# andewx/dieselfluid

Hardware: AMD Instinct MI355X
Metric: M particle-steps/sec, 16M-particle WCSPH dam-break; % HBM roofline (higher is better)
Workload: dtype f32; 1 GPU; WCSPH dam-break, 16003008 particles (n3=252), h=2dx, uniform-grid neighbours, density + pressure/viscosity force + integrate + walls, math=fast; particles=16003008, parallelism=single GPU

## Files before the change

dieselfluid_amd/csrc/kernels_skin.hpp:

```cpp
#pragma once

#include "kernels_tiled.hpp"

namespace dsl {

constexpr int kLEntries = 8;
constexpr int kLMaxChunks = 12;
constexpr int kLMaxEntries = kLMaxChunks * kLEntries - 1;
constexpr int kLBlock = 512;
constexpr unsigned int kLGlobal = 0xffffu;
constexpr float kSkinTauSteps = 16.0f;
constexpr int kLQuads = 14;
static_assert(kTRows * kLQuads <= kLBlock, "one quad per lane");
#ifndef DSL_LIST_WALK
#define DSL_LIST_WALK 2
#endif
constexpr int kListWalk = DSL_LIST_WALK;
constexpr int force_list_waves(bool want_v) { return (kListWalk & 2) != 0 && !want_v ? 6 : 4; }

__global__ void k_skin_decide(SkinState* st) {
  const float d = __builtin_sqrtf(__uint_as_float(st->disp2_bits)) * (1.0f + 1.0e-6f);
  const bool rb = st->force != 0 || !(d <= st->budget);
  st->rebuild = rb ? 1 : 0;
  if (st->unlisted * 64 > st->n_live) st->give_up = 1;
  if (rb) {
    st->ids_sel ^= 1;
    st->n_rebuilds += 1;
    st->unlisted = 0;
    st->fields_own = st->fields_padded = 0u;
    const float vmax = __builtin_sqrtf(__uint_as_float(st->vmax2_bits)) * (1.0f + 1.0e-6f);
    float tau = 0.0f;
    if (st->predict > 0.0f && vmax > 0.0f && vmax < 3.0e38f) tau = fminf(st->predict * st->budget / vmax, kSkinTauSteps * st->dt);
    st->tau = tau;
  }
  st->disp = d;
  st->force = 0;
  st->disp2_bits = 0u;
  st->vmax2_bits = 0u;
  st->n_steps += 1;
  st->history = (st->history << 1) | (rb ? 1u : 0u);
  if (st->n_steps >= 16 && __builtin_popcount(st->history & 0xffffu) >= 5) st->give_up = 1;
}

__device__ __forceinline__ unsigned int pad_entry(const TileMeta& m) { return (unsigned int)(m.row_lds[1] - kTPad) << 4; }

__global__ __launch_bounds__(kLBlock) void k_list_build_v1(DevConsts c, TileGrid tg, const int* __restrict__ desc_of,
                                                        const int* __restrict__ n_tiles, const int* __restrict__ desc,
                                                        const unsigned int* __restrict__ nmask, int mstride,
                                                        uint4* __restrict__ lists, int lstride, SkinState* st,
                                                        SkinGate gate, CSoa3 p, float wide_thr) {
  if (gate.closed()) return;
  __shared__ TileMeta metas[2];
  constexpr int kLStaged = 8;
  __shared__ uint4 held[kLStaged][kLBlock];
  __shared__ unsigned int tile_fields[2];
  const int tid = threadIdx.x;
  if (tid < 2) tile_fields[tid] = 0u;
  TileFeed feed(desc_of, *n_tiles);
  int di = 0;
  bool have = feed.pop(di);
  if (have) tile_meta_store(metas[0], tile_meta_request(desc, di));
  for (int cur = 0; have; cur ^= 1) {
    const TileMeta& m = metas[cur];
    sync_lds();
    have = feed.pop(di);
    int table_word = 0;
    if (have) table_word = tile_meta_request(desc, di);
    const int ntarg = m.tprefix[kTB * kTB];
    const unsigned int pad = pad_entry(m);
    if (m.overflow != 0 && tid == 0) atomicAdd(&st->unlisted, ntarg);
    for_each_target<true, kLBlock>(ntarg, tid, tid, [&](auto shared_c, int t, int sub, int k) {
      constexpr bool SHARED = decltype(shared_c)::value;
      if (SHARED && sub != 0) return;
      const TileTarget tt = tile_target(m, t);
      const int g = tt.g;
      unsigned int b0 = 0u, b1 = 0u, b2 = 0u, b3 = 0u;
      int n = 0;
      auto push = [&](unsigned int entry) {
        b0 = __builtin_amdgcn_alignbit(b1, b0, 16);
        b1 = __builtin_amdgcn_alignbit(b2, b1, 16);
        b2 = __builtin_amdgcn_alignbit(b3, b2, 16);
        b3 = (b3 >> 16) | (entry << 16);
        n += 1;
        if ((n & (kLEntries - 1)) == 0) {
          const int ch = (n >> 3) - 1;
          if (ch < kLStaged) held[ch][tid] = make_uint4(b0, b1, b2, b3);
          else if (ch < kLMaxChunks) lists[(size_t)ch * lstride + g] = make_uint4(b0, b1, b2, b3);
        }
      };
      auto emit = [&](int rec) {
        if (rec != tt.own) push((unsigned int)rec << 4);
      };
      const bool masks = m.overflow == 0;
      if (masks) {
        int rj[9], rje[9];
        unsigned int w1[9], w2[9];
#pragma unroll
        for (int ri = 0; ri < 9; ++ri) {
          tile_run(m, tt.srow + (ri / 3 - 1) * kTH + (ri % 3 - 1), tt.lx, rj[ri], rje[ri]);
          const int len = rje[ri] - rj[ri];
          w1[ri] = (len > 0 && len <= 64) ? nmask[(size_t)ri * mstride + g] : 0u;
          w2[ri] = (len > 32 && len <= 64) ? nmask[(size_t)(kMaskHigh + ri) * mstride + g] : 0u;
        }
        push(0u);
#pragma unroll
        for (int ri = 0; ri < 9; ++ri) {
          const int j = rj[ri], je = rje[ri], len = je - j;
          if (len > 64) {
            const int rr = tt.srow + (ri / 3 - 1) * kTH + (ri % 3 - 1);
            const int g0 = m.row_gs[rr] - m.row_lds[rr];
            const float xi = p.x[g], yi = p.y[g], zi = p.z[g];
            for (int r = j; r < je; ++r) {
              const float dx = xi - p.x[g0 + r], dy = yi - p.y[g0 + r], dz = zi - p.z[g0 + r];
              const float tq = __builtin_fmaf(-dist2<true>(dx, dy, dz), c.inv_hh, 1.0f);
              if (tq > wide_thr) emit(r);
            }
            continue;
          }
          unsigned int w = w1[ri];
          int top = j + ((min(len, 32) + 3) & ~3) - 1;
          while (w != 0u) {
            const int b = __builtin_ctz(w);
            w &= w - 1u;
            emit(top - b);
          }
          w = w2[ri];
          top = j + 32 + ((len - 32 + 3) & ~3) - 1;
          while (w != 0u) {
            const int b = __builtin_ctz(w);
            w &= w - 1u;
            emit(top - b);
          }
        }
      }
      const bool fits = masks && n <= kLMaxChunks * kLEntries;
      if (masks && !fits) st->list_overflow = 1;
      int fields = fits ? n : 0;
      const int own_fields = fields;
      if constexpr (!SHARED) {
        int wmax = 0;
#pragma unroll
        for (int bit = 6; bit >= 0; --bit) {
          const int cand = wmax | (1 << bit);
          if (__builtin_amdgcn_ballot_w64(fields >= cand) != 0ull) wmax = cand;
        }
        fields = wmax;
      }
      atomicAdd(&tile_fields[0], (unsigned int)own_fields);
      atomicAdd(&tile_fields[1], (unsigned int)(fits ? fields : 0));
      const int nch = (fields + kLEntries - 1) / kLEntries;
      if (fits)
        while (n < nch * kLEntries) push(pad);
      for (int ch = 0; ch < min(nch, kLStaged); ++ch) {
        uint4 v = held[ch][tid];
        if (ch == 0) v.x = (v.x & 0xffff0000u) | (unsigned int)fields;
        if (fits) lists[(size_t)ch * lstride + g] = v;
      }
      if (!fits) lists[g] = make_uint4(kLGlobal, 0u, 0u, 0u);
    });
    if (have) tile_meta_store(metas[cur ^ 1], table_word);
    sync_lds();
    if (tid == 0) {
      atomicAdd(&st->fields_own, tile_fields[0]);
      atomicAdd(&st->fields_padded, tile_fields[1]);
      tile_fields[0] = tile_fields[1] = 0u;
    }
  }
}

constexpr int kLQueue = 24;
__global__ __launch_bounds__(kLBlock, 4) void k_list_build(DevConsts c, TileGrid tg, const int* __restrict__ desc_of,
                                                        const int* __restrict__ n_tiles, const int* __restrict__ desc,
                                                        const unsigned int* __restrict__ nmask, int mstride,
                                                        uint4* __restrict__ lists, int lstride, SkinState* st,
                                                        SkinGate gate, CSoa3 p, float wide_thr) {
  if (gate.closed()) return;
  __shared__ TileMeta metas[2];
  __shared__ unsigned int qword[kLQueue][kLBlock];
  __shared__ unsigned short qtop[kLQueue][kLBlock];
  __shared__ unsigned int tile_fields[2];
  const int tid = threadIdx.x;
  if (tid < 2) tile_fields[tid] = 0u;
  TileFeed feed(desc_of, *n_tiles);
  int di = 0;
  bool have = feed.pop(di);
  if (have) tile_meta_store(metas[0], tile_meta_request(desc, di));
  for (int cur = 0; have; cur ^= 1) {
    const TileMeta& m = metas[cur];
    sync_lds();
    have = feed.pop(di);
    int table_word = 0;
    if (have) table_word = tile_meta_request(desc, di);
    const int ntarg = m.tprefix[kTB * kTB];
    const unsigned int pad = pad_entry(m);
    if (m.overflow != 0 && tid == 0) atomicAdd(&st->unlisted, ntarg);
    for_each_target<true, kLBlock>(ntarg, tid, tid, [&](auto shared_c, int t, int sub, int k) {
      constexpr bool SHARED = decltype(shared_c)::value;
      if (SHARED && sub != 0) return;
      const TileTarget tt = tile_target(m, t);
      const int g = tt.g;
      const bool masks = m.overflow == 0;
      int nq = 0, total = 0;
      bool too_many = false;
      auto enqueue = [&](unsigned int w, int top) {
        if (w != 0u) {
          if (nq < kLQueue) {
            qword[nq][tid] = w;
            qtop[nq][tid] = (unsigned short)top;
          } else {
            too_many = true;
          }
          nq += 1;
          total += __builtin_popcount(w);
        }
      };
      if (masks) {
        unsigned int run[9], w1[9], w2[9];
        unsigned int unmasked = 0u;
#pragma unroll
        for (int ri = 0; ri < 9; ++ri) {
          run[ri] = (unsigned int)m.run[(tt.srow + (ri / 3 - 1) * kTH + (ri % 3 - 1)) * kTB + tt.lx - 1];
          const int len = (int)(run[ri] >> 16) - (int)(run[ri] & 0xffffu);
          w1[ri] = (len > 0 && len <= 64) ? nmask[(size_t)ri * mstride + g] : 0u;
          w2[ri] = (len > 32 && len <= 64) ? nmask[(size_t)(kMaskHigh + ri) * mstride + g] : 0u;
          if (len > 64) unmasked |= 1u << ri;
        }
#pragma unroll
        for (int ri = 0; ri < 9; ++ri) {
          const int j = (int)(run[ri] & 0xffffu), len = (int)(run[ri] >> 16) - j;
          unsigned int a = w1[ri], b = w2[ri];
          const int top1 = j + ((min(len, 32) + 3) & ~3) - 1;
          const int top2 = j + 32 + ((len - 32 + 3) & ~3) - 1;
          if (ri == 4) {
            const int b1 = top1 - tt.own, b2 = top2 - tt.own;
            if (b1 >= 0 && b1 < 32) a &= ~(1u << b1);
            if (b2 >= 0 && b2 < 32) b &= ~(1u << b2);
          }
          enqueue(a, top1);
          enqueue(b, top2);
        }
        while (unmasked != 0u) {
          const int ri = __builtin_ctz(unmasked);
          unmasked &= unmasked - 1u;
          const int rr = tt.srow + (ri / 3 - 1) * kTH + (ri % 3 - 1);
          int j, je;
          tile_run(m, rr, tt.lx, j, je);
          const int g0 = m.row_gs[rr] - m.row_lds[rr];
          const float xi = p.x[g], yi = p.y[g], zi = p.z[g];
          for (int r0 = j; r0 < je; r0 += 32) {
            unsigned int w = 0u;
            const int top = r0 + 31;
            for (int r = r0; r < min(r0 + 32, je); ++r) {
              const float dx = xi - p.x[g0 + r], dy = yi - p.y[g0 + r], dz = zi - p.z[g0 + r];
              const float tq = __builtin_fmaf(-dist2<true>(dx, dy, dz), c.inv_hh, 1.0f);
              if (tq > wide_thr && r != tt.own) w |= 1u << (top - r);
            }
            enqueue(w, top);
          }
        }
      }
      const int n_own = 1 + total;
      const bool fits = masks && !too_many && n_own <= kLMaxChunks * kLEntries;
      if (masks && !fits) st->list_overflow = 1;
      int fields = fits ? n_own : 0;
      const int own_fields = fields;
      int wmax = 0;
#pragma unroll
      for (int bit = 6; bit >= 0; --bit) {
        const int cand = wmax | (1 << bit);
        if (__builtin_amdgcn_ballot_w64(fields >= cand) != 0ull) wmax = cand;
      }
      if constexpr (!SHARED) fields = fits ? wmax : 0;
      atomicAdd(&tile_fields[0], (unsigned int)own_fields);
      atomicAdd(&tile_fields[1], (unsigned int)fields);
      const int nch = (fields + kLEntries - 1) / kLEntries;
      const int nch_wave = (wmax + kLEntries - 1) / kLEntries;
      unsigned int b0 = 0u, b1 = 0u, b2 = 0u, b3 = 0u;
      unsigned int k0 = 0u, k1 = 0u, k2 = 0u, k3 = 0u;
      int qi = 0;
      unsigned int w = 0u, top = 0u;
      unsigned int wn = (fits && nq > 0) ? qword[0][tid] : 0u, tn = (fits && nq > 0) ? qtop[0][tid] : 0u;
      const int nq_live = fits ? nq : 0;
      for (int it = 0; it < nch_wave * kLEntries; ++it) {
        unsigned int entry = pad;
        if (it == 0) {
          entry = 0u;
        } else {
          if (w == 0u && qi < nq_live) {
            w = wn;
            top = tn;
            qi += 1;
            if (qi < nq_live) {
              wn = qword[qi][tid];
              tn = qtop[qi][tid];
            }
          }
          if (w != 0u) {
            const int b = __builtin_ctz(w);
            w &= w - 1u;
            entry = (top - (unsigned int)b) << 4;
          }
        }
        b0 = __builtin_amdgcn_alignbit(b1, b0, 16);
        b1 = __builtin_amdgcn_alignbit(b2, b1, 16);
        b2 = __builtin_amdgcn_alignbit(b3, b2, 16);
        b3 = (b3 >> 16) | (entry << 16);
        if ((it & (kLEntries - 1)) == kLEntries - 1) {
          const int ch = it >> 3;
          if (ch == 0) {
            k0 = b0, k1 = b1, k2 = b2, k3 = b3;
          } else if (ch < nch) {
            lists[(size_t)ch * lstride + g] = make_uint4(b0, b1, b2, b3);
          }
        }
      }
      if (fits) lists[g] = make_uint4((k0 & 0xffff0000u) | (unsigned int)fields, k1, k2, k3);
      else lists[g] = make_uint4(kLGlobal, 0u, 0u, 0u);
    });
    if (have) tile_meta_store(metas[cur ^ 1], table_word);
    sync_lds();
    if (tid == 0) {
      atomicAdd(&st->fields_own, tile_fields[0]);
      atomicAdd(&st->fields_padded, tile_fields[1]);
      tile_fields[0] = tile_fields[1] = 0u;
    }
  }
}

template <int NF, bool DEALT, class Load4, class Store>
__device__ __forceinline__ void stage_tile(const TileMeta& m, Load4&& load4, Store&& store) {
  if constexpr (DEALT) {
    const int nq = __builtin_amdgcn_readfirstlane((int)m.qprefix[kTRows]);
    auto pass = [&](int base) {
      StageRegs<NF> sr;
      const StageWhere w = stage_issue_dealt<NF>(m, load4, sr, base + (int)threadIdx.x, nq);
      stage_commit_dealt<NF>(sr, w, store);
    };
    pass(0);
    for (int base = kLBlock; base < nq; base += kLBlock) pass(base);
    stage_pads<NF>(m, store, threadIdx.x);
    return;
  }
  const int t = threadIdx.x, r = t / kLQuads, k = t - r * kLQuads;
  if (r >= kTRows) return;
  const int len = m.row_len[r], gs = m.row_gs[r], ls = m.row_lds[r];
  for (int q = k; 4 * q < len; q += kLQuads) {
    float4 v[NF];
    load4(gs + 4 * q, v);
#pragma unroll
    for (int i = 0; i < 4; ++i) {
      if (4 * q + i < len) {
        float rec[NF];
#pragma unroll
        for (int a = 0; a < NF; ++a) rec[a] = f4_at(v[a], i);
        store(ls + 4 * q + i, rec, true);
      }
    }
  }
  const int npad = m.row_lds[r + 1] - ls - len;
  if (k < npad) {
    float rec[NF];
#pragma unroll
    for (int a = 0; a < NF; ++a) rec[a] = 0.0f;
    store(ls + len + k, rec, false);
  }
}

__device__ __forceinline__ const float4& lds_at(const float4* base, unsigned int byte_offset) {
  return *reinterpret_cast<const float4*>(reinterpret_cast<const char*>(base) + byte_offset);
}

struct Chunk {
  unsigned int x, y, z, w;
};
__device__ __forceinline__ Chunk load_chunk(const uint4* __restrict__ lists, size_t index) {
  const uint4 v = lists[index];
  return Chunk{v.x, v.y, v.z, v.w};
}
__device__ __forceinline__ Chunk pad_chunk(unsigned int pad) {
  const unsigned int w = pad | (pad << 16);
  return Chunk{w, w, w, w};
}
__device__ __forceinline__ unsigned int take_count(Chunk& e, unsigned int pad) {
  const unsigned int cnt = e.x & 0xffffu;
  e.x = (e.x & 0xffff0000u) | pad;
  return cnt;
}
__device__ __forceinline__ void loads_issued() {
  asm volatile("" ::: "memory");
  __builtin_amdgcn_sched_barrier(0);
}
typedef unsigned int ListWords __attribute__((ext_vector_type(4)));
typedef const __attribute__((address_space(1))) ListWords* ListPtr;
__device__ __forceinline__ unsigned long long unknown_pointer(const uint4* p) {
  unsigned long long a = reinterpret_cast<unsigned long long>(p);
  asm volatile("" : "+v"(a));
  return a;
}
__device__ __forceinline__ unsigned long long unknown_pointer_uniform(const uint4* p) {
  unsigned long long a = reinterpret_cast<unsigned long long>(p);
  asm volatile("" : "+s"(a));
  return a;
}
struct ChunkRing {
  Chunk c[3];
  unsigned long long next;
  unsigned long long last;
  int lstride, nch;
  __device__ __forceinline__ ChunkRing(const uint4* __restrict__ lists, int lstride_, int g, int nch_, const Chunk& q0,
                                       const Chunk& q1)
      : next(unknown_pointer(lists + (size_t)2 * lstride_ + g)),
        last(unknown_pointer_uniform(lists + (size_t)max(nch_ - 1, 0) * lstride_ + __builtin_amdgcn_readfirstlane(g))),
        lstride(lstride_), nch(nch_) {
    c[0] = q0;
    c[1] = q1;
  }
  __device__ __forceinline__ void request(int ch) {
    if (ch + 2 >= kLMaxChunks) return;
    const ListWords v = *(ListPtr)(ch + 2 < nch ? next : last);
    c[(ch + 2) % 3] = Chunk{v.x, v.y, v.z, v.w};
    next += (unsigned long long)lstride * sizeof(uint4);
  }
  __device__ __forceinline__ const Chunk& at(int ch) const { return c[ch % 3]; }
};
__device__ __forceinline__ int chunks_of(unsigned int cnt) { return cnt == kLGlobal ? 0 : (int)((cnt + kLEntries) >> 3); }

template <class Body>
__device__ __forceinline__ void walk_shared(const uint4* __restrict__ lists, int lstride, int g, unsigned int pad, int sub,
                                            int k, unsigned int fields, Body&& body) {
  const int nch = fields == kLGlobal ? 0 : (int)((fields + kLEntries - 1) >> 3);
  for (int ch = sub; __builtin_amdgcn_ballot_w64(ch < nch) != 0ull; ch += k) {
    Chunk e = pad_chunk(pad);
    if (ch < nch) e = load_chunk(lists, (size_t)ch * lstride + g);
    if (ch == 0) e.x = (e.x & 0xffff0000u) | pad;
    body(e);
  }
}
__device__ __forceinline__ unsigned int shared_fields(const uint4* __restrict__ lists, int g, int sub) {
  unsigned int f = 0u;
  if (sub == 0) f = lists[g].x & 0xffffu;
  return (unsigned int)__shfl((int)f, (int)((threadIdx.x & (kWave - 1)) - sub), kWave);
}

__global__ __launch_bounds__(kLBlock, 4) void k_density_list(DevConsts c, TileGrid tg, const int* __restrict__ desc_of,
                                                             const int* __restrict__ n_tiles, const int* __restrict__ desc,
                                                             const int* __restrict__ cell_start, const SkinState* st,
                                                             CSoa3 pX, CSoa3 pZ, const uint4* __restrict__ lists,
                                                             int lstride, float* __restrict__ rho,
                                                             float* __restrict__ pterm) {
  __shared__ TileMeta metas[2];
  __shared__ float4 A[kTCap];
  const int tid = threadIdx.x;
  const CSoa3 p = st->rebuild ? pZ : pX;
  TileFeed feed(desc_of, *n_tiles);
  int di = 0;
  bool have = feed.pop(di);
  if (have) tile_meta_store(metas[0], tile_meta_request(desc, di));
  for (int cur = 0; have; cur ^= 1) {
    const TileMeta& m = metas[cur];
    sync_lds();
    have = feed.pop(di);
    int table_word = 0;
    if (have) table_word = tile_meta_request(desc, di);
    const int ntarg = m.tprefix[kTB * kTB];
    const bool staged = m.overflow == 0;
    const unsigned int pad = pad_entry(m);
    Chunk q0 = pad_chunk(pad), q1 = q0;
    const bool first_full = ntarg > kLBlock / 2;
    TileTarget tt0{0, 0, 0, 0};
    const int tperm = (tid & ~(kWave - 1)) + b128_group_slot(tid & (kWave - 1));
    if (first_full && tperm < ntarg) {
      tt0 = tile_target(m, tperm);
      q0 = load_chunk(lists, tt0.g);
      q1 = load_chunk(lists, (size_t)lstride + tt0.g);
    }
    if (staged) stage_tile<3, (kStageDealt & 1) != 0>(m, LoadPos4{p}, StoreTileRecord(A, m, c.inv_hh));
    if (have) tile_meta_store(metas[cur ^ 1], table_word);
    sync_lds();
    for_each_target<true, kLBlock>(ntarg, tid, tperm, [&](auto shared_c, int t, int sub, int k) {
      constexpr bool SHARED = decltype(shared_c)::value;
      TileTarget tt;
      unsigned int fields;
      if constexpr (SHARED) {
        tt = tile_target(m, t);
        fields = shared_fields(lists, tt.g, sub);
      } else {
        if (t == tperm) tt = tt0;
        else {
          tt = tile_target(m, t);
          q0 = load_chunk(lists, tt.g);
          q1 = load_chunk(lists, (size_t)lstride + tt.g);
        }
        fields = take_count(q0, pad);
      }
      const int g = tt.g;
      float acc = 0.0f;
      if (staged && fields != kLGlobal) {
        const float4 me = A[tt.own];
        const float two_hh = 2.0f * c.inv_hh;
        const float sx = two_hh * me.x, sy = two_hh * me.y, sz = two_hh * me.z, a0 = 1.0f + me.w;
        float acc0 = 0.0f, acc1 = 0.0f;
        float4 cq[4];
        auto fetch4 = [&](unsigned int w0, unsigned int w1) {
          cq[0] = lds_at(A, w0 & 0xffffu);
          cq[1] = lds_at(A, w0 >> 16);
          cq[2] = lds_at(A, w1 & 0xffffu);
          cq[3] = lds_at(A, w1 >> 16);
        };
        auto sum4 = [&](const float4 (&r)[4]) {
#pragma unroll
          for (int u = 0; u < 4; ++u) {
            const float q = fma_clamp01(r[u].z, sz, __builtin_fmaf(r[u].y, sy, __builtin_fmaf(r[u].x, sx, r[u].w + a0)));
            if (u & 1) acc1 = __builtin_fmaf(q, q, acc1);
            else acc0 = __builtin_fmaf(q, q, acc0);
          }
        };
        if constexpr (SHARED) {
          walk_shared(lists, lstride, g, pad, sub, k, fields, [&](const Chunk& e) {
            fetch4(e.x, e.y);
            float4 c1[4] = {cq[0], cq[1], cq[2], cq[3]};
            fetch4(e.z, e.w);
            sum4(c1);
            sum4(cq);
          });
        } else {
          const int nf = __builtin_amdgcn_readfirstlane((int)fields), nch = (nf + kLEntries - 1) >> 3;
          const uint4* lp = lists + (size_t)2 * lstride + g;
          Chunk e = q0, e1 = q1;
          fetch4(e.x, e.y);
          for (int ch = 0;;) {
            float4 c1[4] = {cq[0], cq[1], cq[2], cq[3]};
            fetch4(e.z, e.w);
            sum4(c1);
            if (8 * ch + 4 >= nf) break;
            const Chunk en = e1;
            if (ch + 2 < nch) e1 = load_chunk(lp, 0);
            lp += lstride;
            float4 c2[4] = {cq[0], cq[1], cq[2], cq[3]};
            fetch4(en.x, en.y);
            sum4(c2);
            e = en;
            ch += 1;
            if (8 * ch >= nf) break;
          }
        }
        acc = acc0 + acc1;
      } else if (sub == 0) {
        const float xi = p.x[g], yi = p.y[g], zi = p.z[g];
        float a = 0.0f;
        for_each_grid_candidate(c, cell_start, xi, yi, zi, [&](int j) {
          if (j == g) return;
          const float dx = xi - p.x[j], dy = yi - p.y[j], dz = zi - p.z[j];
          const float r2 = dist2<true>(dx, dy, dz);
          if (r2 < c.hh) {
            const float q = __builtin_fmaf(-r2, c.inv_hh, 1.0f);
            a = __builtin_fmaf(q, q, a);
          }
        });
        acc = a;
      }
      if constexpr (SHARED) {
        for (int o = 1; o < k; o <<= 1) acc += __shfl_xor(acc, o, kWave);
        if (sub != 0) return;
      }
      acc *= c.mass * c.A;
      rho[g] = acc;
      const float pr = tait_eos<true>(c, acc, c.eos_d0_grad);
      pterm[g] = acc > 0.0f ? dsl_div<true>(pr, acc * acc) : 0.0f;
    });
  }
}

template <bool WANT_G, bool WANT_V, bool QUEUE>
__global__ __launch_bounds__(kLBlock, force_list_waves(WANT_V)) void k_force_list(DevConsts c, TileGrid tg, const int* __restrict__ desc_of,
                                                           const int* __restrict__ n_tiles, const int* __restrict__ desc,
                                                           const int* __restrict__ cell_start, SkinState* st, CSoa3 pX,
                                                           CSoa3 vX, CSoa3 pZ, CSoa3 vZ, CSoa3 pR, const float* __restrict__ rho,
                                                           const float* __restrict__ pterm,
                                                           const uint4* __restrict__ lists, int lstride, Soa3 pout,
                                                           Soa3 vout, DevStats* stats, int* __restrict__ walk_ctr) {
  __shared__ TileMeta metas[2];
  __shared__ float4 A[kTCap];
  __shared__ float4 B[kTCap];
  __shared__ int feed_slot[2];
  const int tid = threadIdx.x;
  const bool rb = st->rebuild != 0;
  const CSoa3 pin = rb ? pZ : pX, vin = rb ? vZ : vX;
  unsigned int vbits = 0u, fbits = 0u, dbits = 0u;
  typename TileSource<QUEUE>::type feed = TileSource<QUEUE>::make(desc_of, *n_tiles, walk_ctr, feed_slot);
  int di = 0;
  bool have = feed.pop(di);
  if (have) tile_meta_store(metas[0], tile_meta_request(desc, di));
  for (int cur = 0; have; cur ^= 1) {
    const TileMeta& m = metas[cur];
    sync_lds();
    have = feed.pop(di);
    int table_word = 0;
    if (have) table_word = tile_meta_request(desc, di);
    const int ntarg = m.tprefix[kTB * kTB];
    const bool staged = m.overflow == 0;
    const unsigned int pad = pad_entry(m);
    Chunk q0 = pad_chunk(pad), q1 = q0;
    const bool first_full = ntarg > kLBlock / 2;
    TileTarget tt0{0, 0, 0, 0};
    const int tperm = (tid & ~(kWave - 1)) + b128_group_slot(tid & (kWave - 1));
    if (first_full && tperm < ntarg) {
      tt0 = tile_target(m, tperm);
      q0 = load_chunk(lists, tt0.g);
      q1 = load_chunk(lists, (size_t)lstride + tt0.g);
    }
    if (staged)
      stage_tile<8, (kStageDealt & 2) != 0>(
          m,
          [&](int gg, float4* o) {
            o[0] = load4u(pin.x + gg);
            o[1] = load4u(pin.y + gg);
            o[2] = load4u(pin.z + gg);
            o[3] = WANT_G ? load4u(pterm + gg) : make_float4(0.f, 0.f, 0.f, 0.f);
            if constexpr (WANT_V) {
              o[4] = load4u(vin.x + gg);
              o[5] = load4u(vin.y + gg);
              o[6] = load4u(vin.z + gg);
              o[7] = load4u(rho + gg);
            } else {
              o[4] = o[5] = o[6] = o[7] = make_float4(0.f, 0.f, 0.f, 0.f);
            }
          },
          [&](int slot, const float* o, bool real) {
            float4 a = make_float4(kFar, kFar, kFar, 0.f), b = make_float4(0.f, 0.f, 0.f, 0.f);
            if (real && o[0] == o[0] && o[1] == o[1] && o[2] == o[2]) {
              a = make_float4(o[0], o[1], o[2], o[3]);
              if constexpr (WANT_V) b = make_float4(o[4], o[5], o[6], o[7] > 0.0f ? __builtin_amdgcn_rcpf(o[7]) : 0.0f);
            }
            A[slot] = a;
            if constexpr (WANT_V) B[slot] = b;
          });
    if (have) tile_meta_store(metas[cur ^ 1], table_word);
    sync_lds();
    for_each_target<true, kLBlock>(ntarg, tid, tperm, [&](auto shared_c, int t, int sub, int k) {
      constexpr bool SHARED = decltype(shared_c)::value;
      TileTarget tt;
      unsigned int fields;
      if constexpr (SHARED) {
        tt = tile_target(m, t);
        fields = shared_fields(lists, tt.g, sub);
      } else {
        if (t == tperm) tt = tt0;
        else {
          tt = tile_target(m, t);
          q0 = load_chunk(lists, tt.g);
          q1 = load_chunk(lists, (size_t)lstride + tt.g);
        }
        fields = take_count(q0, pad);
      }
      const int g = tt.g;
      float px, py, pz, vx, vy, vz;
      float gx = 0.f, gy = 0.f, gz = 0.f, lx_ = 0.f, ly_ = 0.f, lz_ = 0.f, lw_ = 0.f;
      const bool listed = staged && fields != kLGlobal;
      if (listed) {
        const float4 a = A[tt.own];
        px = a.x, py = a.y, pz = a.z;
        const float pti = WANT_G ? a.w : 0.f;
        if (px == kFar) px = py = pz = __uint_as_float(0x7fc00000u);
        if constexpr (WANT_V) {
          const float4 b = B[tt.own];
          vx = b.x, vy = b.y, vz = b.z;
        } else {
          vx = vin.x[g], vy = vin.y[g], vz = vin.z[g];
        }
        if constexpr (WANT_G || WANT_V) {
          const float ninvh = -c.inv_h;
          auto accum = [&](const float4& ra, const float4& rb2) {
            const float dx = ra.x - px, dyy = ra.y - py, dzz = ra.z - pz;
            float r2 = __builtin_fmaf(dzz, dzz, __builtin_fmaf(dyy, dyy, dx * dx));
            r2 = fmaxf(r2, 1.0e-30f);
            const float rinv = __builtin_amdgcn_rsqf(r2);
            const float dist = r2 * rinv;
            const float q = fma1_clamp01_uniform(dist, ninvh);
            if constexpr (WANT_G) {
              const float kk = (q * q) * (pti + ra.w) * rinv;
              gx = __builtin_fmaf(dx, kk, gx);
              gy = __builtin_fmaf(dyy, kk, gy);
              gz = __builtin_fmaf(dzz, kk, gz);
            }
            if constexpr (WANT_V) {
              const float w = q * rb2.w;
              lx_ = __builtin_fmaf(rb2.x, w, lx_);
              ly_ = __builtin_fmaf(rb2.y, w, ly_);
              lz_ = __builtin_fmaf(rb2.z, w, lz_);
              lw_ += w;
            }
          };
          struct Pair1 {
            float4 a, b;
          };
          auto fetch1 = [&](unsigned int off) {
            Pair1 r;
            r.a = lds_at(A, off);
            r.b = r.a;
            if constexpr (WANT_V) r.b = lds_at(B, off);
            return r;
          };
          if constexpr (SHARED) {
            walk_shared(lists, lstride, g, pad, sub, k, fields, [&](const Chunk& e) {
              const unsigned int w[4] = {e.x, e.y, e.z, e.w};
#pragma unroll
              for (int u = 0; u < 4; ++u) {
                const Pair1 r0 = fetch1(w[u] & 0xffffu), r1 = fetch1(w[u] >> 16);
                accum(r0.a, r0.b);
                accum(r1.a, r1.b);
              }
            });
          } else {
            constexpr bool kStraight = (kListWalk & 2) != 0;
            const int nf = __builtin_amdgcn_readfirstlane((int)fields), nch = (nf + kLEntries - 1) >> 3;
            Pair1 p0 = fetch1(q0.x & 0xffffu), p1 = fetch1(q0.x >> 16);
            auto word = [&](unsigned int next_word) {
              Pair1 cu = p0;
              p0 = fetch1(next_word & 0xffffu);
              if constexpr (kStraight) loads_issued();
              accum(cu.a, cu.b);
              cu = p1;
              p1 = fetch1(next_word >> 16);
              if constexpr (kStraight) loads_issued();
              accum(cu.a, cu.b);
            };
            if constexpr (kStraight) {
              ChunkRing ring(lists, lstride, g, nch, q0, q1);
#pragma unroll
              for (int ch = 0; ch < kLMaxChunks; ++ch) {
                ring.request(ch);
                const Chunk& e = ring.at(ch);
                word(e.y);
                if (8 * ch + 2 >= nf) break;
                word(e.z);
                if (8 * ch + 4 >= nf) break;
                word(e.w);
                if (8 * ch + 6 >= nf) break;
                if (ch + 1 == kLMaxChunks) {
                  accum(p0.a, p0.b);
                  accum(p1.a, p1.b);
                  break;
                }
                word(ring.at(ch + 1).x);
                if (8 * ch + 8 >= nf) break;
              }
            } else {
              const uint4* lp = lists + (size_t)2 * lstride + g;
              Chunk e = q0, e1 = q1;
              for (int ch = 0;;) {
                word(e.y);
                if (8 * ch + 2 >= nf) break;
                word(e.z);
                if (8 * ch + 4 >= nf) break;
                word(e.w);
                if (8 * ch + 6 >= nf) break;
                const Chunk en = e1;
                if (ch + 2 < nch) e1 = load_chunk(lp, 0);
                lp += lstride;
                word(en.x);
                e = en;
                ch += 1;
                if (8 * ch >= nf) break;
              }
            }
          }
        }
      } else {
        px = pin.x[g], py = pin.y[g], pz = pin.z[g];
        vx = vin.x[g], vy = vin.y[g], vz = vin.z[g];
        if (sub == 0) {
          float accG[3] = {0.f, 0.f, 0.f}, accV[3] = {0.f, 0.f, 0.f};
          if constexpr (WANT_G || WANT_V)
            force_sweep<true, WANT_G, WANT_V>(c, grid_neigh(cell_start), g, pin, vin, rho, pterm, accG, accV, nullptr, nullptr);
          gx = accG[0], gy = accG[1], gz = accG[2];
          lx_ = accV[0], ly_ = accV[1], lz_ = accV[2];
        }
      }
      if constexpr (SHARED) {
        for (int o = 1; o < k; o <<= 1) {
          gx += __shfl_xor(gx, o, kWave);
          gy += __shfl_xor(gy, o, kWave);
          gz += __shfl_xor(gz, o, kWave);
          lx_ += __shfl_xor(lx_, o, kWave);
          ly_ += __shfl_xor(ly_, o, kWave);
          lz_ += __shfl_xor(lz_, o, kWave);
          lw_ += __shfl_xor(lw_, o, kWave);
        }
        if (sub != 0) return;
      }
      if (listed) {
        if constexpr (WANT_V) {
          lx_ = __builtin_fmaf(-vx, lw_, lx_);
          ly_ = __builtin_fmaf(-vy, lw_, ly_);
          lz_ = __builtin_fmaf(-vz, lw_, lz_);
        }
        const float sg = -c.B;
        gx *= sg;
        gy *= sg;
        gz *= sg;
        const float sv = c.C * c.mass;
        lx_ *= sv;
        ly_ *= sv;
        lz_ *= sv;
      }
      float fx = c.reset[0], fy = c.reset[1], fz = c.reset[2];
      if constexpr (WANT_G) {
        const float dm = rho[g] * c.mass * c.pressure_sign;
        fx = __builtin_fmaf(gx, dm, fx);
        fy = __builtin_fmaf(gy, dm, fy);
        fz = __builtin_fmaf(gz, dm, fz);
      }
      if constexpr (WANT_V) {
        fx = __builtin_fmaf(lx_, c.mu, fx);
        fy = __builtin_fmaf(ly_, c.mu, fy);
        fz = __builtin_fmaf(lz_, c.mu, fz);
      }
      fx += c.ext[0];
      fy += c.ext[1];
      fz += c.ext[2];
      integrate_core(c, fx, fy, fz, px, py, pz, vx, vy, vz, vbits, fbits);
      {
        const float ex = px - pR.x[g], ey = py - pR.y[g], ez = pz - pR.z[g];
        const unsigned int db = nonneg_bits(__builtin_fmaf(ez, ez, __builtin_fmaf(ey, ey, ex * ex)));
        dbits = db > dbits ? db : dbits;
      }
      pout.x[g] = px;
      pout.y[g] = py;
      pout.z[g] = pz;
      vout.x[g] = vx;
      vout.y[g] = vy;
      vout.z[g] = vz;
    });
  }
  feed.finish();
  wave_atomic_max(&stats->max_vel_bits, vbits);
  wave_atomic_max(&stats->max_f_bits, fbits);
  wave_atomic_max(&st->disp2_bits, dbits);
  wave_atomic_max(&st->vmax2_bits, vbits);
}

}
```

Baseline: 8248 M particle-steps/s.

## Pack neighbour list entries as 12-bit indices, ten per 16-byte chunk

```diff
diff --git a/dieselfluid_amd/csrc/kernels_skin.hpp b/dieselfluid_amd/csrc/kernels_skin.hpp
--- a/dieselfluid_amd/csrc/kernels_skin.hpp
+++ b/dieselfluid_amd/csrc/kernels_skin.hpp
@@ -1,17 +1,15 @@
 #pragma once
 
 #include "kernels_tiled.hpp"
+#include "list_chunk.hpp"
 
 namespace dsl {
 
-constexpr int kLEntries = 8;
-constexpr int kLMaxChunks = 12;
-constexpr int kLMaxEntries = kLMaxChunks * kLEntries - 1;
 constexpr int kLBlock = 512;
-constexpr unsigned int kLGlobal = 0xffffu;
 constexpr float kSkinTauSteps = 16.0f;
 constexpr int kLQuads = 14;
 static_assert(kTRows * kLQuads <= kLBlock, "one quad per lane");
+static_assert((unsigned int)kTCap <= kLIndexLimit && (unsigned int)kTCap * sizeof(float4) <= 65536u, "list fields name every staged record");
 #ifndef DSL_LIST_WALK
 #define DSL_LIST_WALK 2
 #endif
@@ -42,7 +40,8 @@
   if (st->n_steps >= 16 && __builtin_popcount(st->history & 0xffffu) >= 5) st->give_up = 1;
 }
 
-__device__ __forceinline__ unsigned int pad_entry(const TileMeta& m) { return (unsigned int)(m.row_lds[1] - kTPad) << 4; }
+__device__ __forceinline__ unsigned int pad_index(const TileMeta& m) { return (unsigned int)(m.row_lds[1] - kTPad); }
+__device__ __forceinline__ unsigned int pad_entry(const TileMeta& m) { return pad_index(m) << 4; }
 
 __global__ __launch_bounds__(kLBlock) void k_list_build_v1(DevConsts c, TileGrid tg, const int* __restrict__ desc_of,
                                                         const int* __restrict__ n_tiles, const int* __restrict__ desc,
@@ -67,29 +66,29 @@
     int table_word = 0;
     if (have) table_word = tile_meta_request(desc, di);
     const int ntarg = m.tprefix[kTB * kTB];
-    const unsigned int pad = pad_entry(m);
+    const unsigned int pad = pad_index(m);
     if (m.overflow != 0 && tid == 0) atomicAdd(&st->unlisted, ntarg);
     for_each_target<true, kLBlock>(ntarg, tid, tid, [&](auto shared_c, int t, int sub, int k) {
       constexpr bool SHARED = decltype(shared_c)::value;
       if (SHARED && sub != 0) return;
       const TileTarget tt = tile_target(m, t);
       const int g = tt.g;
-      unsigned int b0 = 0u, b1 = 0u, b2 = 0u, b3 = 0u;
+      Chunk b{0u, 0u, 0u, 0u};
       int n = 0;
-      auto push = [&](unsigned int entry) {
-        b0 = __builtin_amdgcn_alignbit(b1, b0, 16);
-        b1 = __builtin_amdgcn_alignbit(b2, b1, 16);
-        b2 = __builtin_amdgcn_alignbit(b3, b2, 16);
-        b3 = (b3 >> 16) | (entry << 16);
+      int pos = 0, ch = 0;
+      auto push = [&](unsigned int index) {
+        chunk_push(b, pos, index);
         n += 1;
-        if ((n & (kLEntries - 1)) == 0) {
-          const int ch = (n >> 3) - 1;
-          if (ch < kLStaged) held[ch][tid] = make_uint4(b0, b1, b2, b3);
-          else if (ch < kLMaxChunks) lists[(size_t)ch * lstride + g] = make_uint4(b0, b1, b2, b3);
+        pos += 1;
+        if (pos == kLEntries) {
+          if (ch < kLStaged) held[ch][tid] = make_uint4(b.x, b.y, b.z, b.w);
+          else if (ch < kLMaxChunks) lists[(size_t)ch * lstride + g] = make_uint4(b.x, b.y, b.z, b.w);
+          pos = 0;
+          ch += 1;
         }
       };
       auto emit = [&](int rec) {
-        if (rec != tt.own) push((unsigned int)rec << 4);
+        if (rec != tt.own) push((unsigned int)rec);
       };
       const bool masks = m.overflow == 0;
       if (masks) {
@@ -133,7 +132,7 @@
           }
         }
       }
-      const bool fits = masks && n <= kLMaxChunks * kLEntries;
+      const bool fits = masks && n <= kLMaxEntries + 1;
       if (masks && !fits) st->list_overflow = 1;
       int fields = fits ? n : 0;
       const int own_fields = fields;
@@ -148,15 +147,19 @@
       }
       atomicAdd(&tile_fields[0], (unsigned int)own_fields);
       atomicAdd(&tile_fields[1], (unsigned int)(fits ? fields : 0));
-      const int nch = (fields + kLEntries - 1) / kLEntries;
+      const int nch = chunks_for(fields);
       if (fits)
         while (n < nch * kLEntries) push(pad);
-      for (int ch = 0; ch < min(nch, kLStaged); ++ch) {
-        uint4 v = held[ch][tid];
-        if (ch == 0) v.x = (v.x & 0xffff0000u) | (unsigned int)fields;
-        if (fits) lists[(size_t)ch * lstride + g] = v;
-      }
-      if (!fits) lists[g] = make_uint4(kLGlobal, 0u, 0u, 0u);
+      for (int hc = 0; hc < min(nch, kLStaged); ++hc) {
+        const uint4 v = held[hc][tid];
+        Chunk e{v.x, v.y, v.z, v.w};
+        if (hc == 0) chunk_set_count(e, (unsigned int)fields);
+        if (fits) lists[(size_t)hc * lstride + g] = make_uint4(e.x, e.y, e.z, e.w);
+      }
+      if (!fits) {
+        const Chunk e = chunk_unlisted();
+        lists[g] = make_uint4(e.x, e.y, e.z, e.w);
+      }
     });
     if (have) tile_meta_store(metas[cur ^ 1], table_word);
     sync_lds();
@@ -192,7 +195,7 @@
     int table_word = 0;
     if (have) table_word = tile_meta_request(desc, di);
     const int ntarg = m.tprefix[kTB * kTB];
-    const unsigned int pad = pad_entry(m);
+    const unsigned int pad = pad_index(m);
     if (m.overflow != 0 && tid == 0) atomicAdd(&st->unlisted, ntarg);
     for_each_target<true, kLBlock>(ntarg, tid, tid, [&](auto shared_c, int t, int sub, int k) {
       constexpr bool SHARED = decltype(shared_c)::value;
@@ -260,7 +263,7 @@
         }
       }
       const int n_own = 1 + total;
-      const bool fits = masks && !too_many && n_own <= kLMaxChunks * kLEntries;
+      const bool fits = masks && !too_many && n_own <= kLMaxEntries + 1;
       if (masks && !fits) st->list_overflow = 1;
       int fields = fits ? n_own : 0;
       const int own_fields = fields;
@@ -273,18 +276,19 @@
       if constexpr (!SHARED) fields = fits ? wmax : 0;
       atomicAdd(&tile_fields[0], (unsigned int)own_fields);
       atomicAdd(&tile_fields[1], (unsigned int)fields);
-      const int nch = (fields + kLEntries - 1) / kLEntries;
-      const int nch_wave = (wmax + kLEntries - 1) / kLEntries;
-      unsigned int b0 = 0u, b1 = 0u, b2 = 0u, b3 = 0u;
-      unsigned int k0 = 0u, k1 = 0u, k2 = 0u, k3 = 0u;
+      const int nch = chunks_for(fields);
+      const int nch_wave = chunks_for(wmax);
+      Chunk b{0u, 0u, 0u, 0u};
+      Chunk k0{0u, 0u, 0u, 0u};
+      int pos = 0, ch = 0;
       int qi = 0;
       unsigned int w = 0u, top = 0u;
       unsigned int wn = (fits && nq > 0) ? qword[0][tid] : 0u, tn = (fits && nq > 0) ? qtop[0][tid] : 0u;
       const int nq_live = fits ? nq : 0;
       for (int it = 0; it < nch_wave * kLEntries; ++it) {
-        unsigned int entry = pad;
+        unsigned int index = pad;
         if (it == 0) {
-          entry = 0u;
+          index = 0u;
         } else {
           if (w == 0u && qi < nq_live) {
             w = wn;
@@ -296,26 +300,26 @@
             }
           }
           if (w != 0u) {
-            const int b = __builtin_ctz(w);
+            const int bit = __builtin_ctz(w);
             w &= w - 1u;
-            entry = (top - (unsigned int)b) << 4;
-          }
-        }
-        b0 = __builtin_amdgcn_alignbit(b1, b0, 16);
-        b1 = __builtin_amdgcn_alignbit(b2, b1, 16);
-        b2 = __builtin_amdgcn_alignbit(b3, b2, 16);
-        b3 = (b3 >> 16) | (entry << 16);
-        if ((it & (kLEntries - 1)) == kLEntries - 1) {
-          const int ch = it >> 3;
+            index = top - (unsigned int)bit;
+          }
+        }
+        chunk_push(b, pos, index);
+        pos += 1;
+        if (pos == kLEntries) {
           if (ch == 0) {
-            k0 = b0, k1 = b1, k2 = b2, k3 = b3;
+            k0 = b;
           } else if (ch < nch) {
-            lists[(size_t)ch * lstride + g] = make_uint4(b0, b1, b2, b3);
-          }
-        }
-      }
-      if (fits) lists[g] = make_uint4((k0 & 0xffff0000u) | (unsigned int)fields, k1, k2, k3);
-      else lists[g] = make_uint4(kLGlobal, 0u, 0u, 0u);
+            lists[(size_t)ch * lstride + g] = make_uint4(b.x, b.y, b.z, b.w);
+          }
+          pos = 0;
+          ch += 1;
+        }
+      }
+      if (fits) chunk_set_count(k0, (unsigned int)fields);
+      else k0 = chunk_unlisted();
+      lists[g] = make_uint4(k0.x, k0.y, k0.z, k0.w);
     });
     if (have) tile_meta_store(metas[cur ^ 1], table_word);
     sync_lds();
@@ -370,21 +374,13 @@
   return *reinterpret_cast<const float4*>(reinterpret_cast<const char*>(base) + byte_offset);
 }
 
-struct Chunk {
-  unsigned int x, y, z, w;
-};
 __device__ __forceinline__ Chunk load_chunk(const uint4* __restrict__ lists, size_t index) {
   const uint4 v = lists[index];
   return Chunk{v.x, v.y, v.z, v.w};
 }
-__device__ __forceinline__ Chunk pad_chunk(unsigned int pad) {
+__device__ __forceinline__ Chunk pad_words(unsigned int pad) {
   const unsigned int w = pad | (pad << 16);
   return Chunk{w, w, w, w};
-}
-__device__ __forceinline__ unsigned int take_count(Chunk& e, unsigned int pad) {
-  const unsigned int cnt = e.x & 0xffffu;
-  e.x = (e.x & 0xffff0000u) | pad;
-  return cnt;
 }
 __device__ __forceinline__ void loads_issued() {
   asm volatile("" ::: "memory");
@@ -423,22 +419,42 @@
   }
   __device__ __forceinline__ const Chunk& at(int ch) const { return c[ch % 3]; }
 };
-__device__ __forceinline__ int chunks_of(unsigned int cnt) { return cnt == kLGlobal ? 0 : (int)((cnt + kLEntries) >> 3); }
-
+__device__ __forceinline__ int chunks_of(unsigned int cnt) { return cnt == kLGlobal ? 0 : chunks_for((int)cnt + 1); }
+
+struct Share {
+  unsigned int w[4];
+};
 template <class Body>
 __device__ __forceinline__ void walk_shared(const uint4* __restrict__ lists, int lstride, int g, unsigned int pad, int sub,
                                             int k, unsigned int fields, Body&& body) {
-  const int nch = fields == kLGlobal ? 0 : (int)((fields + kLEntries - 1) >> 3);
-  for (int ch = sub; __builtin_amdgcn_ballot_w64(ch < nch) != 0ull; ch += k) {
-    Chunk e = pad_chunk(pad);
-    if (ch < nch) e = load_chunk(lists, (size_t)ch * lstride + g);
-    if (ch == 0) e.x = (e.x & 0xffff0000u) | pad;
-    body(e);
+  const int nf = fields == kLGlobal ? 0 : (int)fields;
+  const Chunk far_away = pad_words(pad);
+  for (int v = sub; __builtin_amdgcn_ballot_w64(8 * v < nf) != 0ull; v += k) {
+    Share s{{far_away.x, far_away.y, far_away.z, far_away.w}};
+    if constexpr (kLWords == 4) {
+      if (8 * v < nf) {
+        Chunk e = load_chunk(lists, (size_t)v * lstride + g);
+        if (v == 0) chunk_set_first(e, pad);
+        s = Share{{e.x, e.y, e.z, e.w}};
+      }
+    } else if (8 * v < nf) {
+      const int ch = (4 * v) / kLWords, p = 4 * v - ch * kLWords;
+      Chunk e = load_chunk(lists, (size_t)ch * lstride + g);
+      if (ch == 0) chunk_set_first(e, pad);
+      Chunk f = far_away;
+      if (p > 1 && (ch + 1) * kLEntries < nf) f = load_chunk(lists, (size_t)(ch + 1) * lstride + g);
+      const unsigned int t = chunk_tail(e);
+      s.w[0] = p == 0 ? e.x : p == 1 ? e.y : p == 2 ? e.z : p == 3 ? e.w : t;
+      s.w[1] = p == 0 ? e.y : p == 1 ? e.z : p == 2 ? e.w : p == 3 ? t : f.x;
+      s.w[2] = p == 0 ? e.z : p == 1 ? e.w : p == 2 ? t : p == 3 ? f.x : f.y;
+      s.w[3] = p == 0 ? e.w : p == 1 ? t : p == 2 ? f.x : p == 3 ? f.y : f.z;
+    }
+    body(s);
   }
 }
 __device__ __forceinline__ unsigned int shared_fields(const uint4* __restrict__ lists, int g, int sub) {
   unsigned int f = 0u;
-  if (sub == 0) f = lists[g].x & 0xffffu;
+  if (sub == 0) f = chunk_count(load_chunk(lists, g));
   return (unsigned int)__shfl((int)f, (int)((threadIdx.x & (kWave - 1)) - sub), kWave);
 }
 
@@ -465,7 +481,7 @@
     const int ntarg = m.tprefix[kTB * kTB];
     const bool staged = m.overflow == 0;
     const unsigned int pad = pad_entry(m);
-    Chunk q0 = pad_chunk(pad), q1 = q0;
+    Chunk q0 = pad_words(pad), q1 = q0;
     const bool first_full = ntarg > kLBlock / 2;
     TileTarget tt0{0, 0, 0, 0};
     const int tperm = (tid & ~(kWave - 1)) + b128_group_slot(tid & (kWave - 1));
@@ -502,46 +518,93 @@
         float acc0 = 0.0f, acc1 = 0.0f;
         float4 cq[4];
         auto fetch4 = [&](unsigned int w0, unsigned int w1) {
-          cq[0] = lds_at(A, w0 & 0xffffu);
-          cq[1] = lds_at(A, w0 >> 16);
-          cq[2] = lds_at(A, w1 & 0xffffu);
-          cq[3] = lds_at(A, w1 >> 16);
+          cq[0] = lds_at(A, word_lo(w0));
+          cq[1] = lds_at(A, word_hi(w0));
+          cq[2] = lds_at(A, word_lo(w1));
+          cq[3] = lds_at(A, word_hi(w1));
+        };
+        auto sum1 = [&](const float4& r, bool odd) {
+          const float q = fma_clamp01(r.z, sz, __builtin_fmaf(r.y, sy, __builtin_fmaf(r.x, sx, r.w + a0)));
+          if (odd) acc1 = __builtin_fmaf(q, q, acc1);
+          else acc0 = __builtin_fmaf(q, q, acc0);
         };
         auto sum4 = [&](const float4 (&r)[4]) {
 #pragma unroll
-          for (int u = 0; u < 4; ++u) {
-            const float q = fma_clamp01(r[u].z, sz, __builtin_fmaf(r[u].y, sy, __builtin_fmaf(r[u].x, sx, r[u].w + a0)));
-            if (u & 1) acc1 = __builtin_fmaf(q, q, acc1);
-            else acc0 = __builtin_fmaf(q, q, acc0);
-          }
+          for (int u = 0; u < 4; ++u) sum1(r[u], (u & 1) != 0);
         };
         if constexpr (SHARED) {
-          walk_shared(lists, lstride, g, pad, sub, k, fields, [&](const Chunk& e) {
-            fetch4(e.x, e.y);
+          walk_shared(lists, lstride, g, pad, sub, k, fields, [&](const Share& e) {
+            fetch4(e.w[0], e.w[1]);
             float4 c1[4] = {cq[0], cq[1], cq[2], cq[3]};
-            fetch4(e.z, e.w);
-            sum4(c1);
+            cq[0] = lds_at(A, word_lo(e.w[2]));
+            cq[1] = lds_at(A, word_hi(e.w[2]));
+            sum1(c1[0], false);
+            sum1(c1[1], true);
+            loads_issued();
+            cq[2] = lds_at(A, word_lo(e.w[3]));
+            cq[3] = lds_at(A, word_hi(e.w[3]));
+            sum1(c1[2], false);
+            sum1(c1[3], true);
             sum4(cq);
           });
         } else {
-          const int nf = __builtin_amdgcn_readfirstlane((int)fields), nch = (nf + kLEntries - 1) >> 3;
+          const int nf = __builtin_amdgcn_readfirstlane((int)fields), nch = chunks_for(nf);
           const uint4* lp = lists + (size_t)2 * lstride + g;
           Chunk e = q0, e1 = q1;
-          fetch4(e.x, e.y);
-          for (int ch = 0;;) {
-            float4 c1[4] = {cq[0], cq[1], cq[2], cq[3]};
-            fetch4(e.z, e.w);
-            sum4(c1);
-            if (8 * ch + 4 >= nf) break;
-            const Chunk en = e1;
-            if (ch + 2 < nch) e1 = load_chunk(lp, 0);
-            lp += lstride;
-            float4 c2[4] = {cq[0], cq[1], cq[2], cq[3]};
-            fetch4(en.x, en.y);
-            sum4(c2);
-            e = en;
-            ch += 1;
-            if (8 * ch >= nf) break;
+          if constexpr (kLWords == 5) {
+            auto sum3 = [&](const float4 (&r)[3], bool odd) {
+              sum1(r[0], odd);
+              sum1(r[1], !odd);
+              sum1(r[2], odd);
+            };
+            cq[0] = lds_at(A, word_lo(e.x));
+            cq[1] = lds_at(A, word_hi(e.x));
+            cq[2] = lds_at(A, word_lo(e.y));
+            for (int ch = 0, f0 = 0;;) {
+              float4 c1[3] = {cq[0], cq[1], cq[2]};
+              const unsigned int tail = chunk_tail(e);
+              cq[0] = lds_at(A, word_hi(e.y));
+              cq[1] = lds_at(A, word_lo(e.z));
+              cq[2] = lds_at(A, word_hi(e.z));
+              sum3(c1, false);
+              if (f0 + 3 >= nf) break;
+              float4 c2[3] = {cq[0], cq[1], cq[2]};
+              cq[0] = lds_at(A, word_lo(e.w));
+              cq[1] = lds_at(A, word_hi(e.w));
+              cq[2] = lds_at(A, word_lo_clean(tail));
+              cq[3] = lds_at(A, word_hi_clean(tail));
+              sum3(c2, true);
+              if (f0 + 6 >= nf) break;
+              const Chunk en = e1;
+              if (ch + 2 < nch) e1 = load_chunk(lp, 0);
+              lp += lstride;
+              float4 c3[4] = {cq[0], cq[1], cq[2], cq[3]};
+              cq[0] = lds_at(A, word_lo(en.x));
+              cq[1] = lds_at(A, word_hi(en.x));
+              cq[2] = lds_at(A, word_lo(en.y));
+              sum4(c3);
+              e = en;
+              ch += 1;
+              f0 += kLEntries;
+              if (f0 >= nf) break;
+            }
+          } else {
+            fetch4(e.x, e.y);
+            for (int ch = 0;;) {
+              float4 c1[4] = {cq[0], cq[1], cq[2], cq[3]};
+              fetch4(e.z, e.w);
+              sum4(c1);
+              if (8 * ch + 4 >= nf) break;
+              const Chunk en = e1;
+              if (ch + 2 < nch) e1 = load_chunk(lp, 0);
+              lp += lstride;
+              float4 c2[4] = {cq[0], cq[1], cq[2], cq[3]};
+              fetch4(en.x, en.y);
+              sum4(c2);
+              e = en;
+              ch += 1;
+              if (8 * ch >= nf) break;
+            }
           }
         }
         acc = acc0 + acc1;
@@ -600,7 +663,7 @@
     const int ntarg = m.tprefix[kTB * kTB];
     const bool staged = m.overflow == 0;
     const unsigned int pad = pad_entry(m);
-    Chunk q0 = pad_chunk(pad), q1 = q0;
+    Chunk q0 = pad_words(pad), q1 = q0;
     const bool first_full = ntarg > kLBlock / 2;
     TileTarget tt0{0, 0, 0, 0};
     const int tperm = (tid & ~(kWave - 1)) + b128_group_slot(tid & (kWave - 1));
@@ -702,29 +765,30 @@
             return r;
           };
           if constexpr (SHARED) {
-            walk_shared(lists, lstride, g, pad, sub, k, fields, [&](const Chunk& e) {
-              const unsigned int w[4] = {e.x, e.y, e.z, e.w};
+            walk_shared(lists, lstride, g, pad, sub, k, fields, [&](const Share& e) {
 #pragma unroll
               for (int u = 0; u < 4; ++u) {
-                const Pair1 r0 = fetch1(w[u] & 0xffffu), r1 = fetch1(w[u] >> 16);
+                const Pair1 r0 = fetch1(word_lo(e.w[u])), r1 = fetch1(word_hi(e.w[u]));
                 accum(r0.a, r0.b);
                 accum(r1.a, r1.b);
               }
             });
           } else {
             constexpr bool kStraight = (kListWalk & 2) != 0;
-            const int nf = __builtin_amdgcn_readfirstlane((int)fields), nch = (nf + kLEntries - 1) >> 3;
-            Pair1 p0 = fetch1(q0.x & 0xffffu), p1 = fetch1(q0.x >> 16);
-            auto word = [&](unsigned int next_word) {
+            const int nf = __builtin_amdgcn_readfirstlane((int)fields), nch = chunks_for(nf);
+            Pair1 p0 = fetch1(word_lo(q0.x)), p1 = fetch1(word_hi(q0.x));
+            auto word_of = [&](unsigned int next_word, auto clean) {
               Pair1 cu = p0;
-              p0 = fetch1(next_word & 0xffffu);
+              p0 = fetch1(decltype(clean)::value ? word_lo_clean(next_word) : word_lo(next_word));
               if constexpr (kStraight) loads_issued();
               accum(cu.a, cu.b);
               cu = p1;
-              p1 = fetch1(next_word >> 16);
+              p1 = fetch1(decltype(clean)::value ? word_hi_clean(next_word) : word_hi(next_word));
               if constexpr (kStraight) loads_issued();
               accum(cu.a, cu.b);
             };
+            auto word = [&](unsigned int next_word) { word_of(next_word, std::false_type{}); };
+            auto tail = [&](const Chunk& e) { word_of(chunk_tail(e), std::true_type{}); };
             if constexpr (kStraight) {
               ChunkRing ring(lists, lstride, g, nch, q0, q1);
 #pragma unroll
@@ -732,36 +796,45 @@
                 ring.request(ch);
                 const Chunk& e = ring.at(ch);
                 word(e.y);
-                if (8 * ch + 2 >= nf) break;
+                if (kLEntries * ch + 2 >= nf) break;
                 word(e.z);
-                if (8 * ch + 4 >= nf) break;
+                if (kLEntries * ch + 4 >= nf) break;
                 word(e.w);
-                if (8 * ch + 6 >= nf) break;
+                if (kLEntries * ch + 6 >= nf) break;
+                if constexpr (kLWords == 5) {
+                  tail(e);
+                  if (kLEntries * ch + 8 >= nf) break;
+                }
                 if (ch + 1 == kLMaxChunks) {
                   accum(p0.a, p0.b);
                   accum(p1.a, p1.b);
                   break;
                 }
                 word(ring.at(ch + 1).x);
-                if (8 * ch + 8 >= nf) break;
+                if (kLEntries * ch + kLEntries >= nf) break;
               }
             } else {
               const uint4* lp = lists + (size_t)2 * lstride + g;
               Chunk e = q0, e1 = q1;
-              for (int ch = 0;;) {
+              for (int ch = 0, f0 = 0;;) {
                 word(e.y);
-                if (8 * ch + 2 >= nf) break;
+                if (f0 + 2 >= nf) break;
                 word(e.z);
-                if (8 * ch + 4 >= nf) break;
+                if (f0 + 4 >= nf) break;
                 word(e.w);
-                if (8 * ch + 6 >= nf) break;
+                if (f0 + 6 >= nf) break;
+                if constexpr (kLWords == 5) {
+                  tail(e);
+                  if (f0 + 8 >= nf) break;
+                }
                 const Chunk en = e1;
                 if (ch + 2 < nch) e1 = load_chunk(lp, 0);
                 lp += lstride;
                 word(en.x);
                 e = en;
                 ch += 1;
-                if (8 * ch >= nf) break;
+                f0 += kLEntries;
+                if (f0 >= nf) break;
               }
             }
           }
diff --git a/dieselfluid_amd/csrc/list_chunk.hpp b/dieselfluid_amd/csrc/list_chunk.hpp
--- /dev/null
+++ b/dieselfluid_amd/csrc/list_chunk.hpp
@@ -0,0 +1,79 @@
+#pragma once
+
+#ifndef DSL_LIST_BITS
+#define DSL_LIST_BITS 12
+#endif
+#if DSL_LIST_BITS != 12 && DSL_LIST_BITS != 16
+#error "DSL_LIST_BITS is 12 or 16"
+#endif
+
+#if defined(__HIPCC__) || defined(__CUDACC__)
+#define DSL_CHUNK_FN __host__ __device__ __forceinline__
+#else
+#define DSL_CHUNK_FN inline
+#endif
+
+namespace dsl {
+
+constexpr int kListBits = DSL_LIST_BITS;
+constexpr int kLEntries = kListBits == 12 ? 10 : 8;
+constexpr int kLWords = kLEntries / 2;
+constexpr int kLMaxEntries = 95;
+constexpr int kLMaxChunks = (kLMaxEntries + 1 + kLEntries - 1) / kLEntries;
+constexpr unsigned int kLIndexLimit = 4096u;
+constexpr unsigned int kLGlobal = kListBits == 12 ? 0xfffu : 0xffffu;
+constexpr unsigned int kLOffsetMask = kListBits == 12 ? 0xfff0u : 0xffffu;
+constexpr unsigned int kLNibbles = 0x000f000fu;
+static_assert(kLMaxChunks * kLEntries > kLMaxEntries && (unsigned int)kLMaxEntries + 1u < kLGlobal, "the length fits its field");
+
+struct Chunk {
+  unsigned int x, y, z, w;
+};
+
+DSL_CHUNK_FN unsigned int word_lo(unsigned int w) { return w & kLOffsetMask; }
+DSL_CHUNK_FN unsigned int word_hi(unsigned int w) { return kListBits == 12 ? (w >> 16) & kLOffsetMask : w >> 16; }
+DSL_CHUNK_FN unsigned int word_lo_clean(unsigned int w) { return w & 0xffffu; }
+DSL_CHUNK_FN unsigned int word_hi_clean(unsigned int w) { return w >> 16; }
+DSL_CHUNK_FN unsigned int chunk_tail(const Chunk& e) {
+  const unsigned int r = (e.x & kLNibbles) | ((e.y & kLNibbles) << 4) | ((e.z & kLNibbles) << 8);
+  return r << 4;
+}
+DSL_CHUNK_FN unsigned int chunk_word(const Chunk& e, int p) {
+  return p == 0 ? e.x : p == 1 ? e.y : p == 2 ? e.z : p == 3 ? e.w : chunk_tail(e);
+}
+DSL_CHUNK_FN unsigned int chunk_offset(const Chunk& e, int pos) {
+  const unsigned int w = chunk_word(e, pos >> 1);
+  return (pos & 1) ? word_hi(w) : word_lo(w);
+}
+DSL_CHUNK_FN unsigned int chunk_count(const Chunk& e) { return kListBits == 12 ? (e.x >> 4) & 0xfffu : e.x & 0xffffu; }
+
+DSL_CHUNK_FN void chunk_set_first(Chunk& e, unsigned int offset) {
+  e.x = (e.x & (kListBits == 12 ? 0xffff000fu : 0xffff0000u)) | offset;
+}
+DSL_CHUNK_FN void chunk_set_count(Chunk& e, unsigned int fields) { chunk_set_first(e, kListBits == 12 ? fields << 4 : fields); }
+DSL_CHUNK_FN unsigned int take_count(Chunk& e, unsigned int pad) {
+  const unsigned int cnt = chunk_count(e);
+  chunk_set_first(e, pad);
+  return cnt;
+}
+DSL_CHUNK_FN void chunk_push(Chunk& e, int pos, unsigned int index) {
+  if (kListBits == 16 || pos < 8) {
+    e.x = (e.x >> 16) | (e.y << 16);
+    e.y = (e.y >> 16) | (e.z << 16);
+    e.z = (e.z >> 16) | (e.w << 16);
+    e.w = (e.w >> 16) | (index << 20);
+  } else {
+    const int sh = (pos - 8) * 16;
+    e.x |= (index & 0xfu) << sh;
+    e.y |= ((index >> 4) & 0xfu) << sh;
+    e.z |= ((index >> 8) & 0xfu) << sh;
+  }
+}
+DSL_CHUNK_FN Chunk chunk_unlisted() {
+  Chunk e{0u, 0u, 0u, 0u};
+  chunk_set_count(e, kLGlobal);
+  return e;
+}
+DSL_CHUNK_FN int chunks_for(int fields) { return (fields + kLEntries - 1) / kLEntries; }
+
+}
```

Measured after the change: 8324 M particle-steps/s (median of 6 runs). About the same (+0.9%).
